# RWails/shadow

Hardware: AMD Instinct MI355X
Metric: SSSP source-paths/sec + attached-pair matrix build time; % HBM peak, 1/2/4/8 GPU (higher is better)
Workload: dtype f64

## Files before the change

### include/shadowtopo.h

```cpp
#ifndef SHADOWTOPO_H
#define SHADOWTOPO_H

#include <stddef.h>
#include <stdint.h>

#ifdef __cplusplus
extern "C" {
#endif

typedef struct shadowtopo_engine shadowtopo_engine;

#define SHADOWTOPO_OK 0
#define SHADOWTOPO_EINVAL (-1)
#define SHADOWTOPO_ENOMEM (-2)
#define SHADOWTOPO_EDEVICE (-3)
#define SHADOWTOPO_ESTATE (-4)
#define SHADOWTOPO_EINTERNAL (-5)

#define SHADOWTOPO_F_DIRECTED 0x1u
#define SHADOWTOPO_F_COMPLETE 0x2u
#define SHADOWTOPO_F_PREFER_DIRECT 0x4u
#define SHADOWTOPO_F_SELF_DIJKSTRA_LOOP 0x8u
#define SHADOWTOPO_F_AUTO_COMPLETE 0x10u
#define SHADOWTOPO_F_FORCE_DENSE 0x20u
#define SHADOWTOPO_F_FORCE_CSR 0x40u

#define SHADOWTOPO_MEM_HOST 0
#define SHADOWTOPO_MEM_DEVICE 1
#define SHADOWTOPO_MEM_HOST_LR 2

#define SHADOWTOPO_KIND_NONE 0
#define SHADOWTOPO_KIND_DIRECT 1
#define SHADOWTOPO_KIND_SELF 2
#define SHADOWTOPO_KIND_DIJKSTRA 3

#define SHADOWTOPO_OPT_BATCHES_IN_FLIGHT 1
#define SHADOWTOPO_OPT_TIMING 2
#define SHADOWTOPO_OPT_MAX_ROUNDS 3
#define SHADOWTOPO_OPT_FORCE_REPLAY 4
#define SHADOWTOPO_OPT_PROFILE 5
#define SHADOWTOPO_OPT_DENSE_VARIANT 6
#define SHADOWTOPO_DENSE_F32 0
#define SHADOWTOPO_DENSE_F64 1
#define SHADOWTOPO_OPT_DELTA_PERMILLE 7
#define SHADOWTOPO_OPT_CSR_VARIANT 8
#define SHADOWTOPO_OPT_DENSE_BATCHES_PER_WAVE 9
#define SHADOWTOPO_OPT_SOURCE_ORDER 10
#define SHADOWTOPO_OPT_DENSE_SEED 11
#define SHADOWTOPO_OPT_DENSE_PRUNE 12

#define SHADOWTOPO_OPT_WORKLIST 14
#define SHADOWTOPO_OPT_GRID_X 15
#define SHADOWTOPO_OPT_PRUNE_PENDANT 16
#define SHADOWTOPO_OPT_DEVICE_ROUNDS 17
#define SHADOWTOPO_OPT_DELTA_LIVE 19
#define SHADOWTOPO_OPT_DENSE_W16 20
#define SHADOWTOPO_OPT_SWEEP_PARTS 22
#define SHADOWTOPO_OPT_CHAIN_PARTS 23
#define SHADOWTOPO_OPT_DENSE_SPEC 21
#define SHADOWTOPO_OPT_HEAVY_FIRST 27
#define SHADOWTOPO_OPT_WALK_TPW 28
#define SHADOWTOPO_OPT_CSR_LEAN 30
#define SHADOWTOPO_OPT_CSR_INCREMENTAL 31
#define SHADOWTOPO_OPT_SPEC_COMPOSE 33
#define SHADOWTOPO_OPT_SPIN_US 35
#define SHADOWTOPO_OPT_HOST_GROUPS 36
#define SHADOWTOPO_OPT_SWEEP_STATS 37
#define SHADOWTOPO_OPT_SWEEP_WINDOWS 38
#define SHADOWTOPO_OPT_SWEEP_GLDS 39
#define SHADOWTOPO_OPT_SWEEP_REFILTER 40
#define SHADOWTOPO_OPT_SWEEP_WAVES 41
#define SHADOWTOPO_OPT_SEED_SKIP 42
#define SHADOWTOPO_OPT_DELTA_W16 43
#define SHADOWTOPO_OPT_PART0_PERMILLE 29
#define SHADOWTOPO_OPT_TEST_UNCONVERGED 24
#define SHADOWTOPO_OPT_TEST_SCRAMBLE_TREE 25
#define SHADOWTOPO_OPT_TEST_POOL_ENOMEM 26
#define SHADOWTOPO_OPT_HBM_SHARE 13

#define SHADOWTOPO_CSR_FULL 1
#define SHADOWTOPO_CSR_PUSH 2

typedef struct shadowtopo_stats {
    int64_t n_vertices;
    int64_t n_edges;
    int64_t n_arcs;
    int64_t n_attached;
    int64_t sources;
    int64_t batches;
    int64_t rounds;
    int64_t relax_launches;
    int64_t replayed_sources;
    int64_t tainted_pairs;
    double relax_ms;
    double compose_ms;
    double replay_ms;
    double wall_ms;
    int32_t device;
    int32_t multigraph;
    int32_t dense;
    int32_t reserved;
    int64_t visits;
    int64_t changes;
    int64_t full_sweeps;
    int64_t delta_sweeps;
    double full_ms;
    double delta_ms;
    int64_t full_batches;
    int64_t full_changes;
    int64_t relax_batches;
    int64_t wl_launches;
    double wl_ms;
    int64_t sparse_deltas;
    double self_ms;
    int64_t self_paths;
    int64_t pruned_deltas;
    int64_t pruned_vertices;
    int64_t pool_allocs;
    double pool_alloc_ms;
    double create_validate_ms;
    double create_upload_ms;
    double create_build_ms;
    double order_ms;
    double create_alloc_ms;
// ... 76 lines not shown
```

### shadow_amd/csrc/engine.hip

```cpp
#include <hip/hip_runtime.h>
#include <sys/mman.h>

#include <algorithm>
#include <atomic>
#include <chrono>
#include <cmath>
#include <cstdarg>
#include <cstdint>
#include <cstdlib>
#include <cstdio>
#include <cstring>
#include <functional>
#include <limits>
#include <mutex>
#include <string>
#include <thread>
#include <type_traits>
#include <vector>

#include "graph_build.h"
#include "shadowtopo.h"

namespace {

// ... 1499 lines not shown
                    int nr = 0;
#pragma unroll
                    for (int x = 0; x < XR; ++x) {
                        rp[x] = u0;
                        if (hrows) {
                            rp[x] = u0 + __builtin_ctzll(hrows);
                            hrows &= hrows - 1;
                            nr = x + 1;
                        }
                        ur[x] = PR ? perm[rp[x]] : rp[x];
                    }
                    double d64[XR], ws[XR][TDT];
#pragma unroll
                    for (int x = 0; x < XR; ++x) {
                        d64[x] = (lpass >> (rp[x] - u0)) & 1ull ? Dl[(size_t)ur[x] * KL] : dinf();
#pragma unroll
                        for (int t = 0; t < TDT; ++t) ws[x][t] = W[(size_t)rp[x] * Vp + v0 + t];
                    }
#pragma unroll
                    for (int x = 0; x < XR; ++x) {
                        if (x >= nr) break;
                        const int32_t u = ur[x];
                        const bool own = (u == sv[k]);
#pragma unroll
                        for (int t = 0; t < TDT; ++t) {
                            const double c = d64[x] + ws[x][t];
                            if (__ballot((c <= bc[k][t]) & !own)) {
                                if (!own) lex_update(c, d64[x], u, bc[k][t], bdu[k][t], bu[k][t], tie[k], 1u << t);
                            }
                        }
                    }
                }
            }
        }
    }
    if (v0 < V) {
#pragma unroll
        for (int k = 0; k < TB; ++k)
            if (live[k])
            {
                SeedRows sr;
                if (PR && WIp && sv[k] >= 0) {
                    sr.WIp = WIp;
                    sr.WRp = WRp;
                    sr.srow = (size_t)ipos[sv[k]] * Vp;
                    sr.rs = vfac[sv[k]];
                }
                dense_epilogue<TDT>(B[k], lane, sv[k], v0, V, bc[k], bdu[k], bu[k], tie[k], WI, Vp, in_r, parity,
                                    cnt, b0 + k, vid, sr,
                                    mdc_out ? mdc_out + ((size_t)(b0 + k) * (Vp / KL) + v0 / KL) * KL : nullptr,
                                    seeded != 0);
            }
    }
}

constexpr int HEAVY_MAX = 2048;
struct HeavyArgs {
    const uint32_t* w[4];
    int32_t* o[4];
    int32_t slots[4];
};
__global__ __launch_bounds__(1024) void k_heavy_order(HeavyArgs ha) {
    __shared__ unsigned long long key[HEAVY_MAX];
    const int x = blockIdx.x, part = blockIdx.y;
    const int32_t S = ha.slots[part];
    if (S <= 0) return;
    const uint32_t* w = ha.w[part];
    int32_t* ord = ha.o[part];
    int n2 = 1;
    while (n2 < S) n2 <<= 1;
    for (int j = threadIdx.x; j < n2; j += blockDim.x)
        key[j] = j < S ? ((unsigned long long)w[8 * j + x] << 32) | (uint32_t)(0xffffffffu - (uint32_t)j) : 0ull;
    __syncthreads();
    for (int k = 2; k <= n2; k <<= 1)
        for (int jj = k >> 1; jj > 0; jj >>= 1) {
            for (int i = threadIdx.x; i < n2; i += blockDim.x) {
                const int l = i ^ jj;
                if (l > i) {
                    const unsigned long long a = key[i], b = key[l];
                    const bool desc = (i & k) == 0;
                    if (desc ? a < b : a > b) {
                        key[i] = b;
                        key[l] = a;
                    }
                }
            }
            __syncthreads();
        }
    for (int r = threadIdx.x; r < S; r += blockDim.x) {
        const int32_t j = (int32_t)(0xffffffffu - (uint32_t)key[r]);
        ord[8 * r + x] = 8 * j + x;
    }
}

template <typename T>
__global__ __launch_bounds__(256) void k_permute_w(const T* __restrict__ W, const int32_t* __restrict__ perm,
                                                   int32_t Vp, T* __restrict__ Wp) {
    const size_t i = blockIdx.x;
    const __attribute__((address_space(1))) T* src = (const __attribute__((address_space(1))) T*)W + (size_t)perm[i] * Vp;
    for (int32_t j = threadIdx.x; j < Vp; j += 256) Wp[i * Vp + j] = src[perm[j]];
}

__global__ __launch_bounds__(256) void k_w16(const float* __restrict__ W32p, uint16_t* __restrict__ W16p, size_t n) {
    for (size_t i = (size_t)blockIdx.x * blockDim.x + threadIdx.x; i < n; i += (size_t)gridDim.x * blockDim.x) {
        const float f = W32p[i];
        uint16_t hb;
// ... 1430 lines not shown
    void* stage = nullptr;
    size_t stage_bytes = 0;
    hipStream_t copy_stream = nullptr;
    hipEvent_t ev_comp[2] = {nullptr, nullptr}, ev_copy[2] = {nullptr, nullptr};
    ReplayDev rp{};
    bool rp_ready = false;
    std::vector<void*> rp_allocs;
    int32_t opt_nb = 0;
    int32_t opt_timing = 0;
    int64_t opt_max_rounds = 0;
    int32_t opt_force_replay = 0;
    int32_t opt_profile = 0;
    int32_t opt_dense_variant = 0;
    int32_t opt_dense_tb = 1;
    int32_t opt_delta_permille = 125;
    int32_t opt_hbm_share = 1000;
    bool floor_ok = false;
    bool floor_checked = false;
    size_t pool_bytes = 0;
    int32_t opt_worklist = 1;
    int32_t opt_csr_variant = SHADOWTOPO_CSR_FULL;
    int32_t trace_rounds = 0;
    int32_t opt_delta_live = 2;
    int32_t opt_delta_live_div = 64;
    int32_t opt_delta_colbound = 2;
    int32_t opt_sweep_spiral = 1;
    int32_t opt_sweep_win1 = 8;
    int32_t opt_sweep_split = 1;
    int32_t opt_sweep_parts = 2;
    hipStream_t aux_stream[3] = {nullptr, nullptr, nullptr};
    hipEvent_t ev_h0 = nullptr, ev_hp[3] = {nullptr, nullptr, nullptr};
    hipEvent_t ev_sw[4] = {nullptr, nullptr, nullptr, nullptr};
    int32_t opt_chain_parts = 1;
    int32_t opt_fuse_mindc = 1;
    int32_t opt_part0_permille = 562;
    int32_t opt_host_split = 4;
    int64_t opt_grid_x = (int64_t)1 << 23;
    int32_t* d_live = nullptr;
    int32_t* d_nlive = nullptr;
    unsigned long long* d_prof = nullptr;
    unsigned long long* prof_buf = nullptr;
    hipEvent_t ev0 = nullptr, ev1 = nullptr, evm = nullptr, evm2 = nullptr;
    hipEvent_t ev_spin = nullptr;
    std::vector<hipEvent_t> ev_dev;
    std::vector<hipEvent_t> ev_spec;
    void* d_pk_scratch = nullptr;
    size_t pk_scratch_n = 0;
    int32_t* h_cnt_spec = nullptr;
    int32_t opt_dense_spec = 2;
    int32_t opt_sweep_glds = 0;
    int32_t opt_sweep_stats = 0;
    unsigned long long* d_sweep_hits = nullptr;
    int32_t opt_sweep_waves = 4;
    int32_t opt_sweep_refilter = 0;
    int32_t opt_seed_skip = 1;
    int32_t opt_delta_w16 = 1;
    float* d_thrio = nullptr;
    size_t thrio_n = 0;
    int32_t opt_heavy_first = 1;
    int32_t opt_csr_lean = 2;
    bool lean_next = false;
    ViewBufs vb;
    size_t view_cap_a = 0;
    int32_t opt_host_groups = 0;
    int32_t opt_spin_us = 20000;
    int32_t opt_spec_compose = 1;
    unsigned long long* h_masks = nullptr;
    size_t h_masks_n = 0;
    int32_t opt_csr_incremental = 32;
    int32_t opt_walk_tpw = 1;
    uint32_t* d_bweight[4] = {nullptr, nullptr, nullptr, nullptr};
    int32_t* d_border[4][2] = {};
    size_t heavy_cap[4] = {0, 0, 0, 0};
    int64_t heavy_key[4] = {-1, -1, -1, -1};
    int64_t heavy_next[4] = {-1, -1, -1, -1};
    int heavy_buf = 0;
    int32_t opt_test_unconverged = 0;
    int32_t opt_test_scramble = 0;
    int32_t opt_test_pool_enomem = 0;
    bool unconverged = false;
    shadowtopo_stats st{};
};

namespace {

int dev_alloc(std::vector<void*>& owner, void** p, size_t bytes) {
    if (bytes == 0) bytes = 8;
    hipError_t e = hipMalloc(p, bytes);
    if (e != hipSuccess) return fail(SHADOWTOPO_ENOMEM, "hipMalloc(%zu): %s", bytes, hipGetErrorString(e));
    owner.push_back(*p);
    return SHADOWTOPO_OK;
}

template <typename T>
int upload(shadowtopo_engine* eng, const std::vector<T>& h, const T** out) {
    void* p = nullptr;
    int rc = dev_alloc(eng->graph_allocs, &p, h.size() * sizeof(T));
    if (rc) return rc;
    if (!h.empty()) HIP_TRY(hipMemcpy(p, h.data(), h.size() * sizeof(T), hipMemcpyHostToDevice));
    *out = static_cast<const T*>(p);
    return SHADOWTOPO_OK;
}

float f32_round_down(double x) {
    float f = (float)x;
    if ((double)f > x) f = std::nextafter(f, -std::numeric_limits<float>::infinity());
// ... 214 lines not shown
                           float* mdc_out, int32_t seeded) {
    constexpr int TDT = FTDT, XR = 2;
    const int32_t ntb = (eng->V + 4 * TDT - 1) / (4 * TDT);
    const int32_t ngroups = (nbg + TB - 1) / TB;
    const int64_t nblocks = 8 * (((int64_t)ngroups * ntb + 7) / 8);
    const size_t nchunks = (size_t)((eng->V + SRS - 1) / SRS);
    const size_t need = (size_t)ngroups * (size_t)(eng->Vp / TDT) * TB * nchunks;
    if (eng->hitlog_n < need) {
        if (eng->d_hitlog) (void)hipFree(eng->d_hitlog);
        eng->d_hitlog = nullptr;
        eng->hitlog_n = 0;
        hipError_t e = hipMalloc((void**)&eng->d_hitlog, need * sizeof(uint32_t));
        if (e != hipSuccess) return e;
        eng->hitlog_n = need;
    }
    if (eng->vperm_ready && eng->opt_dense_prune) {
        const size_t mneed = (size_t)eng->nb_cap * nchunks * KL;
        if (eng->minD_n < mneed) {
            if (eng->d_minD) (void)hipFree(eng->d_minD);
            eng->d_minD = nullptr;
            eng->minD_n = 0;
            hipError_t e = hipMalloc((void**)&eng->d_minD, mneed * sizeof(float));
            if (e != hipSuccess) return e;
            eng->minD_n = mneed;
        }
        hipLaunchKernelGGL(k_min_d32, dim3((uint32_t)((nchunks + 3) / 4), nbg), dim3(256), 0, s, eng->pools,
                           eng->d_perm, (int32_t)nchunks, eng->d_minD);
        if (TB <= 2 && eng->opt_sweep_split) {
            if (eng->opt_dense_w16) {
                hipError_t e = ensure_w16p(eng, s);
                if (e != hipSuccess) return e;
            }
            bool w16 = false;
            if constexpr (TB == 1 && TDT == 8) {
                w16 = eng->opt_dense_w16 != 0;
                if (w16)
                    hipLaunchKernelGGL((k_relax_dense_f<TDT, XR, TB, true, 1, 4, true>), dim3((uint32_t)nblocks), dim3(256),
                                       0, s, (const float*)eng->d_W16p, eng->d_Wp, eng->d_WI, eng->Vp, eng->g.in_r,
                                       eng->pools, eng->V, nbg, ntb, par, thresh, cnt_prev, cnt_cur, eng->d_prof,
                                       eng->d_hitlog, eng->d_perm, eng->d_minW, eng->d_minD, eng->d_pos, eng->d_WIp,
                                       eng->d_WRp, eng->g.vfac, eng->opt_sweep_spiral, eng->opt_sweep_win1, nullptr);
            }
            if constexpr (TB == 1) {
                const int32_t parts = sweep_parts(eng, nbg);
                if (!w16 && parts >= 2 && !eng->d_prof) {
                    hipError_t e = hipSuccess;
                    if (!eng->ev_h0) e = hipEventCreateWithFlags(&eng->ev_h0, hipEventDisableTiming);
                    for (int k = 0; k < parts - 1 && e == hipSuccess; ++k) {
                        if (!eng->aux_stream[k]) e = hipStreamCreateWithFlags(&eng->aux_stream[k], hipStreamNonBlocking);
                        if (e == hipSuccess && !eng->ev_hp[k]) e = hipEventCreateWithFlags(&eng->ev_hp[k], hipEventDisableTiming);
                    }
                    if (e == hipSuccess && mdc_out)
                        e = hipMemsetD32Async((hipDeviceptr_t)mdc_out, 0x7fc00000, (size_t)nbg * (eng->Vp / KL) * KL, s);
                    if (e == hipSuccess) e = hipEventRecord(eng->ev_h0, s);
                    for (int k = 0; k < parts - 1 && e == hipSuccess; ++k) e = hipStreamWaitEvent(eng->aux_stream[k], eng->ev_h0, 0);
                    if (e != hipSuccess) return e;
                    if (eng->opt_sweep_stats && !eng->d_sweep_hits &&
                        (e = hipMalloc((void**)&eng->d_sweep_hits, 2 * sizeof(unsigned long long))) != hipSuccess)
                        return e;
                    if (eng->opt_sweep_stats && (e = hipMemsetAsync(eng->d_sweep_hits, 0, 2 * sizeof(unsigned long long), s)) != hipSuccess)
                        return e;
                    if (eng->opt_sweep_refilter) {
                        const size_t need_t = (size_t)nbg * eng->Vp * KL;
                        if (eng->thrio_n < need_t) {
                            if (eng->d_thrio) (void)hipFree(eng->d_thrio);
                            eng->d_thrio = nullptr;
                            eng->thrio_n = 0;
                            if ((e = hipMalloc((void**)&eng->d_thrio, need_t * sizeof(float))) != hipSuccess) return e;
                            eng->thrio_n = need_t;
                        }
                    }
                    const int cur = eng->heavy_buf;
                    HeavyArgs ha{};
                    bool sort_any = false;
                    auto part = [&](hipStream_t st, int32_t b0, int32_t n, int k) {
                        const Pools P = pools_from(eng->pools, b0);
                        uint32_t* hl = eng->d_hitlog + (size_t)b0 * (size_t)(eng->Vp / TDT) * nchunks;
                        const float* mD = eng->d_minD + (size_t)b0 * nchunks * KL;
                        const int64_t nbl = 8 * (((int64_t)n * ntb + 7) / 8);
                        const bool w8 = eng->opt_sweep_waves == 8;
                        const int32_t ntb1 = w8 ? (eng->V + 8 * TDT - 1) / (8 * TDT) : ntb;
                        const int64_t nbl1 = 8 * (((int64_t)n * ntb1 + 7) / 8);
                        const int64_t key = ((int64_t)b0 << 42) | ((int64_t)n << 21) | ((int64_t)w8 << 20) | ntb1;
                        bool heavy = eng->opt_heavy_first && k < 4 && nbl1 / 8 <= HEAVY_MAX;
                        if (heavy && eng->heavy_cap[k] < (size_t)nbl1) {
                            for (void* q : {(void*)eng->d_bweight[k], (void*)eng->d_border[k][0], (void*)eng->d_border[k][1]})
                                if (q) (void)hipFree(q);
                            eng->d_bweight[k] = nullptr;
                            eng->d_border[k][0] = eng->d_border[k][1] = nullptr;
                            eng->heavy_cap[k] = 0;
                            eng->heavy_key[k] = -1;
                            if (hipMalloc((void**)&eng->d_bweight[k], sizeof(uint32_t) * nbl1) != hipSuccess ||
                                hipMalloc((void**)&eng->d_border[k][0], sizeof(int32_t) * nbl1) != hipSuccess ||
                                hipMalloc((void**)&eng->d_border[k][1], sizeof(int32_t) * nbl1) != hipSuccess ||
                                hipMemsetAsync(eng->d_bweight[k], 0, sizeof(uint32_t) * nbl1, st) != hipSuccess) {
                                (void)hipGetLastError();
                                heavy = false;
                            } else {
                                eng->heavy_cap[k] = (size_t)nbl1;
                            }
                        }
                        const int32_t* ord = heavy && eng->heavy_key[k] == key ? eng->d_border[k][cur] : nullptr;
                        float* tio = eng->opt_sweep_refilter ? eng->d_thrio + (size_t)b0 * eng->Vp * KL : nullptr;
                        if (w8 && eng->opt_sweep_glds)
                            hipLaunchKernelGGL((k_relax_dense_f<TDT, XR, 1, true, 1, 8, false, true>), dim3((uint32_t)nbl1),
                                               dim3(512), 0, st, eng->d_W32p, eng->d_Wp, eng->d_WI, eng->Vp, eng->g.in_r,
                                               P, eng->V, n, ntb1, par, thresh, cnt_prev + b0, cnt_cur + b0, nullptr, hl,
                                               eng->d_perm, eng->d_minW, mD, eng->d_pos, eng->d_WIp, eng->d_WRp,
                                               eng->g.vfac, eng->opt_sweep_spiral, eng->opt_sweep_win1, nullptr, ord,
                                               heavy ? eng->d_bweight[k] : nullptr, tio);
                        else if (w8)
                            hipLaunchKernelGGL((k_relax_dense_f<TDT, XR, 1, true, 1, 8, false, false>), dim3((uint32_t)nbl1),
                                               dim3(512), 0, st, eng->d_W32p, eng->d_Wp, eng->d_WI, eng->Vp, eng->g.in_r,
                                               P, eng->V, n, ntb1, par, thresh, cnt_prev + b0, cnt_cur + b0, nullptr, hl,
                                               eng->d_perm, eng->d_minW, mD, eng->d_pos, eng->d_WIp, eng->d_WRp,
                                               eng->g.vfac, eng->opt_sweep_spiral, eng->opt_sweep_win1, nullptr, ord,
                                               heavy ? eng->d_bweight[k] : nullptr, tio);
                        else if (eng->opt_sweep_glds)
                            hipLaunchKernelGGL((k_relax_dense_f<TDT, XR, 1, true, 1, 4, false, true>), dim3((uint32_t)nbl),
                                               dim3(256), 0, st, eng->d_W32p, eng->d_Wp, eng->d_WI, eng->Vp, eng->g.in_r,
                                               P, eng->V, n, ntb, par, thresh, cnt_prev + b0, cnt_cur + b0, nullptr, hl,
                                               eng->d_perm, eng->d_minW, mD, eng->d_pos, eng->d_WIp, eng->d_WRp,
                                               eng->g.vfac, eng->opt_sweep_spiral, eng->opt_sweep_win1, nullptr, ord,
                                               heavy ? eng->d_bweight[k] : nullptr, tio);
                        else
                        hipLaunchKernelGGL((k_relax_dense_f<TDT, XR, 1, true, 1>), dim3((uint32_t)nbl), dim3(256), 0, st,
                                           eng->d_W32p, eng->d_Wp, eng->d_WI, eng->Vp, eng->g.in_r, P, eng->V, n, ntb,
                                           par, thresh, cnt_prev + b0, cnt_cur + b0, nullptr, hl, eng->d_perm,
                                           eng->d_minW, mD, eng->d_pos, eng->d_WIp, eng->d_WRp, eng->g.vfac,
                                           eng->opt_sweep_spiral, eng->opt_sweep_win1, nullptr, ord,
                                           heavy ? eng->d_bweight[k] : nullptr, tio);
                        if (heavy) {
                            ha.w[k] = eng->d_bweight[k];
                            ha.o[k] = eng->d_border[k][cur ^ 1];
                            ha.slots[k] = (int32_t)(nbl1 / 8);
                            eng->heavy_next[k] = key;
                            sort_any = true;
                        } else {
                            eng->heavy_next[k] = -1;
                        }
                        hipLaunchKernelGGL((k_relax_dense_f<TDT, XR, 1, true, 2>), dim3((uint32_t)nbl), dim3(256), 0, st,
                                           eng->d_W32p, eng->d_Wp, eng->d_WI, eng->Vp, eng->g.in_r, P, eng->V, n, ntb,
                                           par, thresh, cnt_prev + b0, cnt_cur + b0,
                                           eng->opt_sweep_stats ? eng->d_sweep_hits : nullptr, hl, eng->d_perm,
                                           eng->d_minW, mD, eng->d_pos, eng->d_WIp, eng->d_WRp, eng->g.vfac,
                                           eng->opt_sweep_spiral, eng->opt_sweep_win1,
                                           mdc_out ? mdc_out + (size_t)b0 * (eng->Vp / KL) * KL : nullptr, nullptr,
                                           nullptr, tio, seeded);
                        if (tail && e == hipSuccess) e = (*tail)(st, b0, n, k);
                    };
                    auto bound = [&](int k) {
                        if (parts == 2 && k == 1 && eng->opt_part0_permille > 0)
                            return std::max<int32_t>(1, std::min<int32_t>(nbg - 1, (int32_t)(((int64_t)nbg * eng->opt_part0_permille + 500) / 1000)));
                        return (int32_t)((int64_t)nbg * k / parts);
                    };
                    for (int k = 0; k < parts; ++k) {
                        const int32_t b0 = bound(k), b1 = bound(k + 1);
                        part(k == 0 ? s : eng->aux_stream[k - 1], b0, b1 - b0, k);
                    }
                    if (sort_any && e == hipSuccess) {
                        hipLaunchKernelGGL(k_heavy_order, dim3(8, (uint32_t)std::min(parts, 4)), dim3(1024), 0, s, ha);
                        for (int k = 0; k < 4; ++k) eng->heavy_key[k] = k < parts ? eng->heavy_next[k] : -1;
                        eng->heavy_buf = cur ^ 1;
                    }
                    for (int k = 0; k < parts - 1 && e == hipSuccess; ++k) {
                        e = hipEventRecord(eng->ev_hp[k], eng->aux_stream[k]);
                        if (e == hipSuccess) e = hipStreamWaitEvent(s, eng->ev_hp[k], 0);
                    }
                    if (e != hipSuccess) return e;
                    if (eng->opt_sweep_stats && sort_any) {
                        if ((e = hipStreamSynchronize(s)) != hipSuccess) return e;
                        for (int k = 0; k < parts && k < 4; ++k) {
                            if (!ha.w[k]) continue;
                            std::vector<uint32_t> wk((size_t)ha.slots[k] * 8);
                            if ((e = hipMemcpy(wk.data(), ha.w[k], wk.size() * sizeof(uint32_t), hipMemcpyDeviceToHost)) != hipSuccess)
                                return e;
                            for (uint32_t x : wk) eng->st.sweep_chunks += x;
                            const int32_t ntbs = eng->opt_sweep_waves == 8 ? (eng->V + 8 * TDT - 1) / (8 * TDT) : ntb;
                            eng->st.sweep_chunk_slots += (int64_t)(bound(k + 1) - bound(k)) * ntbs * (int64_t)nchunks;
                        }
                        unsigned long long hits = 0;
                        if ((e = hipMemcpy(&hits, eng->d_sweep_hits, sizeof hits, hipMemcpyDeviceToHost)) != hipSuccess) return e;
                        eng->st.sweep_hit_rows += (int64_t)hits;
                    }
                    return hipGetLastError();
                }
            }
            if (!w16)
            hipLaunchKernelGGL((k_relax_dense_f<TDT, XR, TB, true, 1>), dim3((uint32_t)nblocks), dim3(256), 0, s,
                               eng->d_W32p, eng->d_Wp, eng->d_WI, eng->Vp, eng->g.in_r, eng->pools, eng->V, nbg, ntb,
                               par, thresh, cnt_prev, cnt_cur, eng->d_prof, eng->d_hitlog, eng->d_perm, eng->d_minW,
                               eng->d_minD, eng->d_pos, eng->d_WIp, eng->d_WRp, eng->g.vfac, eng->opt_sweep_spiral,
                               eng->opt_sweep_win1, nullptr);
            const int64_t nblocks1 = 8 * (((int64_t)nbg * ntb + 7) / 8);
            hipLaunchKernelGGL((k_relax_dense_f<TDT, XR, 1, true, 2>), dim3((uint32_t)nblocks1), dim3(256), 0, s,
                               eng->d_W32p, eng->d_Wp, eng->d_WI, eng->Vp, eng->g.in_r, eng->pools, eng->V, nbg, ntb,
                               par, thresh, cnt_prev, cnt_cur, eng->d_prof, eng->d_hitlog, eng->d_perm, eng->d_minW,
                               eng->d_minD, eng->d_pos, eng->d_WIp, eng->d_WRp, eng->g.vfac, eng->opt_sweep_spiral,
                               eng->opt_sweep_win1, nullptr, nullptr, nullptr, nullptr, seeded);
            return hipGetLastError();
        }
        hipLaunchKernelGGL((k_relax_dense_f<TDT, XR, TB, true>), dim3((uint32_t)nblocks), dim3(256), 0, s,
                           eng->d_W32p, eng->d_Wp, eng->d_WI, eng->Vp, eng->g.in_r, eng->pools, eng->V, nbg, ntb, par,
                           thresh, cnt_prev, cnt_cur, eng->d_prof, eng->d_hitlog, eng->d_perm, eng->d_minW,
                           eng->d_minD, eng->d_pos, eng->d_WIp, eng->d_WRp, eng->g.vfac, eng->opt_sweep_spiral,
                               eng->opt_sweep_win1, nullptr);
        return hipGetLastError();
    }
    hipLaunchKernelGGL((k_relax_dense_f<TDT, XR, TB, false>), dim3((uint32_t)nblocks), dim3(256), 0, s, eng->d_W32,
                       eng->d_W, eng->d_WI, eng->Vp, eng->g.in_r, eng->pools, eng->V, nbg, ntb, par, thresh, cnt_prev,
                       cnt_cur, eng->d_prof, eng->d_hitlog, nullptr, nullptr, nullptr, nullptr, nullptr, nullptr, nullptr, 0, 0, nullptr);
    return hipGetLastError();
}

hipError_t launch_dense_f(shadowtopo_engine* eng, int32_t nbg, int32_t par, int32_t thresh,
                          const int32_t* cnt_prev, int32_t* cnt_cur, hipStream_t s, const PartTail* tail = nullptr,
                          float* mdc_out = nullptr, bool seeded = false) {
    const int32_t sd = seeded && eng->opt_seed_skip;
    switch (eng->opt_dense_tb) {
        case 1: return launch_dense_ft<1>(eng, nbg, par, thresh, cnt_prev, cnt_cur, s, tail, mdc_out, sd);
        case 4: return launch_dense_ft<4>(eng, nbg, par, thresh, cnt_prev, cnt_cur, s, tail, mdc_out, sd);
        default: return launch_dense_ft<2>(eng, nbg, par, thresh, cnt_prev, cnt_cur, s, tail, mdc_out, sd);
    }
}

bool delta_is_sparse(const shadowtopo_engine* eng, int32_t nbg, int32_t thresh) {
    if (eng->opt_delta_live != 2) return eng->opt_delta_live == 1;
    int64_t dch = 0, dpairs = 0;
    for (int32_t b = 0; b < nbg; ++b)
        if (eng->h_cnt[b] > 0 && eng->h_cnt[b] <= thresh) {
            dch += eng->h_cnt[b];
// ... 2047 lines not shown
        case SHADOWTOPO_OPT_SWEEP_PARTS:
            if (value < 1 || value > 4) return fail(SHADOWTOPO_EINVAL, "sweep parts must be 1 .. 4");
            eng->opt_sweep_parts = (int32_t)value;
            return SHADOWTOPO_OK;
        case SHADOWTOPO_OPT_DENSE_SPEC:
            if (value < 0 || value > SPEC_MAX) return fail(SHADOWTOPO_EINVAL, "dense spec rounds must be in [0, 4]");
            eng->opt_dense_spec = (int32_t)value;
            return SHADOWTOPO_OK;
        case SHADOWTOPO_OPT_DELTA_LIVE:
            if (value < 0 || value > 2) return fail(SHADOWTOPO_EINVAL, "delta live must be 0, 1 or 2");
            eng->opt_delta_live = (int32_t)value;
            return SHADOWTOPO_OK;
        case SHADOWTOPO_OPT_WORKLIST:
            if (value < 0 || value > 2) return fail(SHADOWTOPO_EINVAL, "worklist must be 0, 1 or 2");
            eng->opt_worklist = (int32_t)value;
            return SHADOWTOPO_OK;
        case SHADOWTOPO_OPT_HBM_SHARE:
            if (value < 1 || value > 1000) return fail(SHADOWTOPO_EINVAL, "HBM share must be in [1, 1000] per mille");
            eng->opt_hbm_share = (int32_t)value;
            return SHADOWTOPO_OK;
        case SHADOWTOPO_OPT_CSR_LEAN:
            if (value < 0 || value > 2) return fail(SHADOWTOPO_EINVAL, "CSR lean must be 0, 1 or 2");
            eng->opt_csr_lean = (int32_t)value;
            return SHADOWTOPO_OK;
        case SHADOWTOPO_OPT_HOST_GROUPS:
            if (value < 0 || value > 1024) return fail(SHADOWTOPO_EINVAL, "host groups must be in [0, 1024]");
            eng->opt_host_groups = (int32_t)value;
            return SHADOWTOPO_OK;
        case SHADOWTOPO_OPT_SWEEP_WINDOWS:
            if (value < 0 || (value & 0xff) >= 64 || ((value >> 8) & 0xff) >= 64 || value >= (1 << 16))
                return fail(SHADOWTOPO_EINVAL, "sweep windows: bits 0-7 and 8-15 must each be in [0, 63]");
            eng->opt_sweep_win1 = (int32_t)value;
            return SHADOWTOPO_OK;
        case SHADOWTOPO_OPT_SWEEP_GLDS:
            if (value != 0 && value != 1) return fail(SHADOWTOPO_EINVAL, "sweep glds must be 0 or 1");
            eng->opt_sweep_glds = (int32_t)value;
            return SHADOWTOPO_OK;
        case SHADOWTOPO_OPT_SWEEP_WAVES:
            if (value != 4 && value != 8) return fail(SHADOWTOPO_EINVAL, "sweep waves must be 4 or 8");
            eng->opt_sweep_waves = (int32_t)value;
            return SHADOWTOPO_OK;
        case SHADOWTOPO_OPT_DELTA_W16:
            if (value != 0 && value != 1) return fail(SHADOWTOPO_EINVAL, "delta w16 must be 0 or 1");
            eng->opt_delta_w16 = (int32_t)value;
            return SHADOWTOPO_OK;
        case SHADOWTOPO_OPT_SEED_SKIP:
            if (value != 0 && value != 1) return fail(SHADOWTOPO_EINVAL, "seed skip must be 0 or 1");
            eng->opt_seed_skip = (int32_t)value;
            return SHADOWTOPO_OK;
        case SHADOWTOPO_OPT_SWEEP_REFILTER:
            if (value != 0 && value != 1) return fail(SHADOWTOPO_EINVAL, "sweep refilter must be 0 or 1");
            eng->opt_sweep_refilter = (int32_t)value;
            return SHADOWTOPO_OK;
        case SHADOWTOPO_OPT_SWEEP_STATS:
            eng->opt_sweep_stats = value ? 1 : 0;
            return SHADOWTOPO_OK;
        case SHADOWTOPO_OPT_SPIN_US:
            if (value < 0 || value > 10000000) return fail(SHADOWTOPO_EINVAL, "spin must be in [0, 1e7] us");
            eng->opt_spin_us = (int32_t)value;
            return SHADOWTOPO_OK;
        case SHADOWTOPO_OPT_SPEC_COMPOSE:
            if (value != 0 && value != 1) return fail(SHADOWTOPO_EINVAL, "speculative compose must be 0 or 1");
            eng->opt_spec_compose = (int32_t)value;
            return SHADOWTOPO_OK;
        case SHADOWTOPO_OPT_CSR_INCREMENTAL:
            if (value < 0 || value > (1 << 20)) return fail(SHADOWTOPO_EINVAL, "CSR incremental must be in [0, 2^20]");
            eng->opt_csr_incremental = (int32_t)value;
            return SHADOWTOPO_OK;
        case SHADOWTOPO_OPT_PART0_PERMILLE:
            if (value < 1 || value > 999) return fail(SHADOWTOPO_EINVAL, "part 0 share must be in [1, 999] per mille");
            eng->opt_part0_permille = (int32_t)value;
            return SHADOWTOPO_OK;
        case SHADOWTOPO_OPT_WALK_TPW:
            if (value < 1 || value > 4) return fail(SHADOWTOPO_EINVAL, "walk shape must be 1 .. 4");
            eng->opt_walk_tpw = (int32_t)value;
            return SHADOWTOPO_OK;
        case SHADOWTOPO_OPT_HEAVY_FIRST:
            if (value != 0 && value != 1) return fail(SHADOWTOPO_EINVAL, "heavy first must be 0 or 1");
            eng->opt_heavy_first = (int32_t)value;
            return SHADOWTOPO_OK;
        case SHADOWTOPO_OPT_TEST_UNCONVERGED:
            eng->opt_test_unconverged = value ? 1 : 0;
            return SHADOWTOPO_OK;
        case SHADOWTOPO_OPT_TEST_POOL_ENOMEM:
            eng->opt_test_pool_enomem = value ? 1 : 0;
            return SHADOWTOPO_OK;
        case SHADOWTOPO_OPT_TEST_SCRAMBLE_TREE:
            if (value < 0 || value > 2) return fail(SHADOWTOPO_EINVAL, "scramble mode must be 0, 1 or 2");
            eng->opt_test_scramble = (int32_t)value;
            return SHADOWTOPO_OK;
        case SHADOWTOPO_OPT_DELTA_PERMILLE:
            if (value < 0 || value > 1000) return fail(SHADOWTOPO_EINVAL, "delta per mille must be in [0, 1000]");
            eng->opt_delta_permille = (int32_t)value;
            return SHADOWTOPO_OK;
        default:
            return fail(SHADOWTOPO_EINVAL, "unknown option %d", key);
    }
}

int shadowtopo_compute_rows(shadowtopo_engine* eng, int32_t row_begin, int32_t row_end, double* lat, double* rel,
                            uint32_t* hops, uint8_t* kind, int32_t mem, void* stream) {
    if (!eng) return fail(SHADOWTOPO_EINVAL, "NULL engine");
    if (!eng->d_attached) return fail(SHADOWTOPO_ESTATE, "shadowtopo_set_attached not called");
    if (row_begin < 0 || row_end > eng->A || row_begin > row_end) return fail(SHADOWTOPO_EINVAL, "bad row range");
    if (row_begin == row_end) return SHADOWTOPO_OK;
    if (mem != SHADOWTOPO_MEM_HOST && mem != SHADOWTOPO_MEM_DEVICE && mem != SHADOWTOPO_MEM_HOST_LR)
// ... 478 lines not shown
```

### shadow_amd/engine.py

```python
from __future__ import annotations

import ctypes
import os

import numpy as np

HERE = os.path.dirname(os.path.abspath(__file__))
LIB_PATH = os.environ.get("SHADOWTOPO_EXP_LIB") or os.path.join(HERE, "_build", "libshadowtopo_hip.so")

F_DIRECTED = 0x1
F_COMPLETE = 0x2
F_PREFER_DIRECT = 0x4
F_SELF_DIJKSTRA_LOOP = 0x8
F_AUTO_COMPLETE = 0x10
F_FORCE_DENSE = 0x20
F_FORCE_CSR = 0x40

MEM_HOST = 0
MEM_DEVICE = 1
MEM_HOST_LR = 2

KIND_NONE, KIND_DIRECT, KIND_SELF, KIND_DIJKSTRA = 0, 1, 2, 3

OPT_BATCHES_IN_FLIGHT = 1
OPT_TIMING = 2
OPT_MAX_ROUNDS = 3
OPT_FORCE_REPLAY = 4
OPT_PROFILE = 5
OPT_DENSE_VARIANT = 6
DENSE_F32 = 0
DENSE_F64 = 1
OPT_DELTA_PERMILLE = 7
OPT_CSR_VARIANT = 8
OPT_DENSE_BATCHES_PER_WAVE = 9
OPT_SOURCE_ORDER = 10
OPT_DENSE_SEED = 11
OPT_DENSE_PRUNE = 12
OPT_HBM_SHARE = 13
OPT_WORKLIST = 14
OPT_GRID_X = 15
OPT_PRUNE_PENDANT = 16
OPT_DEVICE_ROUNDS = 17
OPT_DENSE_W16 = 20
OPT_CHAIN_PARTS = 23
OPT_SWEEP_PARTS = 22
OPT_DENSE_SPEC = 21
OPT_DELTA_LIVE = 19
OPT_WALK_TPW = 28
OPT_CSR_LEAN = 30
OPT_CSR_INCREMENTAL = 31
OPT_SPEC_COMPOSE = 33
OPT_SPIN_US = 35
OPT_HOST_GROUPS = 36
OPT_SWEEP_WINDOWS = 38
OPT_SWEEP_GLDS = 39
OPT_SWEEP_REFILTER = 40
OPT_SWEEP_WAVES = 41
OPT_DELTA_W16 = 43
OPT_SEED_SKIP = 42
OPT_SWEEP_STATS = 37
OPT_PART0_PERMILLE = 29
OPT_HEAVY_FIRST = 27
OPT_TEST_UNCONVERGED = 24
OPT_TEST_SCRAMBLE_TREE = 25
OPT_TEST_POOL_ENOMEM = 26
CSR_FULL = 1
CSR_PUSH = 2

ENGINE_SYMBOLS = (
    "shadowtopo_device_count", "shadowtopo_prepare", "shadowtopo_last_error", "shadowtopo_create", "shadowtopo_destroy",
    "shadowtopo_set_attached", "shadowtopo_set_option", "shadowtopo_compute_rows", "shadowtopo_sssp",
    "shadowtopo_get_stats", "shadowtopo_reset_stats", "shadowtopo_is_complete", "shadowtopo_get_eid",
    "shadowtopo_host_alloc", "shadowtopo_host_free", "shadowtopo_self_rule_paths",
    "shadowtopo_packed_capacity", "shadowtopo_pack_rows", "shadowtopo_unpack_rows",
    "shadowtopo_hops_narrow", "shadowtopo_hops_widen",
)


class ShadowTopoError(RuntimeError):
    pass


class Stats(ctypes.Structure):
    _fields_ = [
        ("n_vertices", ctypes.c_int64), ("n_edges", ctypes.c_int64), ("n_arcs", ctypes.c_int64),
        ("n_attached", ctypes.c_int64), ("sources", ctypes.c_int64), ("batches", ctypes.c_int64),
        ("rounds", ctypes.c_int64), ("relax_launches", ctypes.c_int64), ("replayed_sources", ctypes.c_int64),
        ("tainted_pairs", ctypes.c_int64), ("relax_ms", ctypes.c_double), ("compose_ms", ctypes.c_double),
        ("replay_ms", ctypes.c_double), ("wall_ms", ctypes.c_double), ("device", ctypes.c_int32),
        ("multigraph", ctypes.c_int32), ("dense", ctypes.c_int32), ("reserved", ctypes.c_int32),
        ("visits", ctypes.c_int64), ("changes", ctypes.c_int64),
        ("full_sweeps", ctypes.c_int64), ("delta_sweeps", ctypes.c_int64),
        ("full_ms", ctypes.c_double), ("delta_ms", ctypes.c_double),
        ("full_batches", ctypes.c_int64), ("full_changes", ctypes.c_int64), ("relax_batches", ctypes.c_int64),
        ("wl_launches", ctypes.c_int64), ("wl_ms", ctypes.c_double), ("sparse_deltas", ctypes.c_int64),
        ("self_ms", ctypes.c_double), ("self_paths", ctypes.c_int64), ("pruned_deltas", ctypes.c_int64),
        ("pruned_vertices", ctypes.c_int64), ("pool_allocs", ctypes.c_int64), ("pool_alloc_ms", ctypes.c_double),
        ("create_validate_ms", ctypes.c_double), ("create_upload_ms", ctypes.c_double),
        ("create_build_ms", ctypes.c_double), ("order_ms", ctypes.c_double),
        ("create_alloc_ms", ctypes.c_double), ("groups", ctypes.c_int64),
        ("prepare_ms", ctypes.c_double), ("create_prepare_wait_ms", ctypes.c_double),
        ("group_batches", ctypes.c_int64), ("host_syncs", ctypes.c_int64),
        ("push_ms", ctypes.c_double), ("pred_ms", ctypes.c_double), ("fold_ms", ctypes.c_double),
        ("push_rounds", ctypes.c_int64), ("fold_rounds", ctypes.c_int64),
        ("packed_pairs", ctypes.c_int64), ("packed_explicit", ctypes.c_int64),
        ("compose_kernel_ms", ctypes.c_double), ("walk_targets", ctypes.c_int64),
        ("attach_prep_ms", ctypes.c_double), ("lean_groups", ctypes.c_int64),
        ("spec_composes", ctypes.c_int64), ("spec_composes_lost", ctypes.c_int64),
        ("sweep_chunks", ctypes.c_int64), ("sweep_chunk_slots", ctypes.c_int64), ("sweep_hit_rows", ctypes.c_int64),
# ... 247 lines not shown
```

Baseline: 333,300.

## Add destination-lane dense sweep kernel mapping lanes to destinations by default

Adds a new dense sweep kernel in which each wave lane owns a destination vertex and loops over a few sources, instead of lanes over sources. Blocks cover 32 sources by 64 destinations, with W and D chunks double-buffered in LDS and chunk-level pruning done through ballots. The aim is to skip more chunk work by changing the shape of the live region and to raise reuse of W rows per wave. It is enabled by default through a new option; the hit log now has to be zeroed before each sweep, and the new kernel uses different threshold, register and LDS behaviour.

After: 372,600, median of 6. +11.8%, better.

```diff
diff --git a/_exp/sweep_lane_shape_sim.py b/_exp/sweep_lane_shape_sim.py
--- /dev/null
+++ b/_exp/sweep_lane_shape_sim.py
@@ -0,0 +1,113 @@
+import sys
+
+import numpy as np
+
+sys.path.insert(0, ".")
+from shadow_amd import synth
+
+V = int(sys.argv[1]) if len(sys.argv) > 1 else 10_000
+A = V // 10
+SRS, KL = 32, 64
+nb = (A + KL - 1) // KL
+BATCHES = [int(x) for x in sys.argv[2].split(",")] if len(sys.argv) > 2 else sorted({0, nb // 2, nb - 2 if nb > 2 else nb - 1})
+
+
+def hilbert(x, y, n=1 << 12):
+    x = (x * (n - 1)).astype(np.int64)
+    y = (y * (n - 1)).astype(np.int64)
+    dd = np.zeros_like(x)
+    s = n >> 1
+    while s > 0:
+        rx = ((x & s) > 0).astype(np.int64)
+        ry = ((y & s) > 0).astype(np.int64)
+        dd += s * s * ((3 * rx) ^ ry)
+        m = ry == 0
+        f = m & (rx == 1)
+        x = np.where(f, n - 1 - x, x)
+        y = np.where(f, n - 1 - y, y)
+        x2 = np.where(m, y, x)
+        y = np.where(m, x, y)
+        x = x2
+        s >>= 1
+    return dd
+
+
+g = synth.geometric_complete_ish(V=V, A=A)
+pts = np.random.default_rng(1).random((V, 2))
+perm = np.argsort(hilbert(pts[:, 0], pts[:, 1]), kind="stable")
+pos = np.empty(V, np.int64)
+pos[perm] = np.arange(V)
+W = np.full((V, V), np.inf, np.float32)
+src, dst = pos[np.asarray(g.src)], pos[np.asarray(g.dst)]
+lat = np.asarray(g.latency, np.float32)
+keep = src != dst
+W[src[keep], dst[keep]] = lat[keep]
+if not g.directed:
+    W = np.minimum(W, W.T)
+att = np.sort(pos[np.asarray(g.attached)])
+nchunks = (V + SRS - 1) // SRS
+Vc = nchunks * SRS
+Vt = (V + KL - 1) // KL * KL
+Wr = np.full((Vc, V), np.inf, np.float32)
+Wr[:V] = W
+minW = Wr.reshape(nchunks, SRS, V).min(1)
+del Wr
+
+
+def min_plus(D):
+    out = D.copy()
+    tmp = np.empty((1024, V), np.float32)
+    for s in range(D.shape[0]):
+        for u0 in range(0, V, 1024):
+            n = min(1024, V - u0)
+            np.add(W[u0:u0 + n], D[s, u0:u0 + n, None], out=tmp[:n])
+            np.minimum(out[s], tmp[:n].min(0), out=out[s])
+    return out
+
+
+SHAPES = [("wave 64 x 8, block 64 x 32 (source lanes)", 64, 8, 64, 32),
+          ("wave 8 x 64, block 32 x 64 (destination lanes)", 8, 64, 32, 64),
+          ("wave 16 x 32", 16, 32, None, None),
+          ("wave 32 x 16", 32, 16, None, None),
+          ("single pairs (floor of any box bound)", 1, 1, None, None)]
+acc = {name: [0, 0, 0, 0] for name, *_ in SHAPES}
+for b in BATCHES:
+    S = att[b * KL:(b + 1) * KL]
+    ns = len(S)
+    D0 = np.full((KL, V), np.inf, np.float32)
+    D0[:ns] = W[S]
+    thr = D0.copy()
+    thr[np.arange(ns), S] = 0.0
+    thr = min_plus(min_plus(thr))
+    thr[np.arange(ns), S] = -np.inf
+    thr[ns:] = -np.inf
+    D0r = np.full((KL, Vc), np.inf, np.float32)
+    D0r[:, :V] = D0
+    minD = D0r.reshape(KL, nchunks, SRS).min(2)
+    thr_p = np.full((KL, Vt), -np.inf, np.float32)
+    thr_p[:, :V] = thr * np.float32(1 + 1e-6)
+    minW_p = np.full((nchunks, Vt), np.inf, np.float32)
+    minW_p[:, :V] = minW
+    live = np.empty((nchunks, KL, Vt), bool)
+    for c in range(nchunks):
+        live[c] = minD[:, c, None] + minW_p[c][None, :] <= thr_p
+    ntiles = {gt: (V + gt - 1) // gt for gt in (1, 8, 16, 32, 64)}
+    for name, gs, gt, bs, bt in SHAPES:
+        w = live.reshape(nchunks, KL // gs, gs, Vt // gt, gt).any(axis=(2, 4))[:, :, :ntiles[gt]]
+        acc[name][0] += int(w.sum())
+        acc[name][1] += w.size
+        if bs:
+            bl = live.reshape(nchunks, KL // bs, bs, Vt // bt, bt).any(axis=(2, 4))[:, :, :ntiles[bt]]
+            acc[name][2] += int(bl.sum())
+            acc[name][3] += bl.size
+    print(f"batch {b}: {ns} sources done", file=sys.stderr, flush=True)
+
+print(f"C2 generator, V = {V}, A = {A}, batches {BATCHES} of {nb}, every tile, {nchunks} chunks of {SRS} rows")
+print(f"{'shape (sources x destinations)':50s} {'live (wave, chunk)':>19s} {'live (block, chunk)':>20s} {'waves per staged chunk':>23s}")
+for name, *_ in SHAPES:
+    lw, sw, lb, sb = acc[name]
+    fw = lw / sw
+    if sb:
+        print(f"{name:50s} {fw:19.3f} {lb / sb:20.3f} {fw / (lb / sb):23.2f}")
+    else:
+        print(f"{name:50s} {fw:19.3f}")
diff --git a/include/shadowtopo.h b/include/shadowtopo.h
--- a/include/shadowtopo.h
+++ b/include/shadowtopo.h
@@ -70,6 +70,7 @@
 #define SHADOWTOPO_OPT_SWEEP_GLDS 39
 #define SHADOWTOPO_OPT_SWEEP_REFILTER 40
 #define SHADOWTOPO_OPT_SWEEP_WAVES 41
+#define SHADOWTOPO_OPT_SWEEP_LANES 44
 #define SHADOWTOPO_OPT_SEED_SKIP 42
 #define SHADOWTOPO_OPT_DELTA_W16 43
 #define SHADOWTOPO_OPT_PART0_PERMILLE 29
diff --git a/shadow_amd/csrc/engine.hip b/shadow_amd/csrc/engine.hip
--- a/shadow_amd/csrc/engine.hip
+++ b/shadow_amd/csrc/engine.hip
@@ -1575,6 +1575,252 @@
                                     seeded != 0);
             }
     }
+}
+
+__global__ __launch_bounds__(256) __attribute__((amdgpu_waves_per_eu(6))) void k_sweep_dest_lanes(
+    const float* __restrict__ W32p, const double* __restrict__ Wp, int32_t Vp, Pools pools, int32_t V, int32_t nb,
+    int32_t ntl, int32_t thresh, const int32_t* __restrict__ cnt_prev, uint32_t* __restrict__ hitlog,
+    const int32_t* __restrict__ perm, const float* __restrict__ minW, const float* __restrict__ minD,
+    const int32_t* __restrict__ ipos, int32_t spiral, int32_t win1, const int32_t* __restrict__ border,
+    uint32_t* __restrict__ bweight) {
+    constexpr int NT = 256, SO = 8;
+    constexpr int BS = 32, BD = 64;
+    struct SweepLds {
+        float d[2][SRS * BS];
+        float w[2][SRS * BD];
+        unsigned long long win[2];
+    };
+    __shared__ __attribute__((aligned(16))) SweepLds slds;
+    auto& sD = slds.d;
+    auto& sW = slds.w;
+    auto& sWin = slds.win;
+    const int64_t Lb = border ? (int64_t)border[blockIdx.x] : (int64_t)blockIdx.x;
+    int32_t b, it;
+    if (!xcd_tile(Lb, nb, 2 * ntl, b, it)) return;
+    const int32_t h = it & 1, t0 = (it >> 1) * BD;
+    if (!(cnt_prev[b] > thresh) || t0 >= V) {
+        if (bweight && threadIdx.x == 0) bweight[Lb] = 0u;
+        return;
+    }
+    const int32_t wave = __builtin_amdgcn_readfirstlane(threadIdx.x >> 6);
+    const int lane = threadIdx.x & 63;
+    const int32_t s0 = BS * h + SO * wave;
+    const int32_t p = t0 + lane;
+    const BatchDev B = batch_view(pools, b);
+    float thr[SO];
+    {
+        const int32_t v = perm[p];
+        double cd[SO];
+#pragma unroll
+        for (int j = 0; j < SO; ++j) cd[j] = B.D[(size_t)v * KL + s0 + j];
+#pragma unroll
+        for (int j = 0; j < SO; ++j) {
+            const int32_t sj = B.srcv[s0 + j];
+            const double ws = (sj >= 0 && sj != v) ? Wp[(size_t)ipos[sj >= 0 ? sj : 0] * Vp + p] : dinf();
+            const double bc = ws < dinf() ? 0.0 + ws : dmax();
+            thr[j] = sj >= 0 && p < V ? f32_thr(cd[j] < bc ? cd[j] : bc) : __int_as_float(0x7fc00000);
+        }
+    }
+    const int32_t nrows = (V + SRS - 1) / SRS * SRS;
+    const int32_t nchunks = nrows / SRS;
+    typedef float f4 __attribute__((ext_vector_type(4)));
+    typedef __attribute__((address_space(1))) const f4 gf4;
+    constexpr int WQ = BD / 4;
+    constexpr int DQ4 = BS / 4;
+    constexpr int WQT = SRS * WQ / NT;
+    static_assert(SRS * DQ4 == NT && WQT * NT == SRS * WQ, "one D32 piece and whole W32p pieces per thread");
+    f4 pd, pw[WQT];
+    float mdn[SO], mdc[SO], mwn, mwc;
+    const gfloat* mDb = (const gfloat*)minD + (size_t)b * nchunks * KL + s0;
+    const gfloat* mWl = (const gfloat*)minW + p;
+    const int32_t c0 = (int32_t)((int64_t)t0 / SRS % nchunks);
+    const int32_t sL = c0, sR = nchunks - 1 - c0, sM = sL < sR ? sL : sR;
+    auto chunk_of = [&](int32_t j) {
+        if (!spiral) return (c0 + j) % nchunks;
+        if (j <= 2 * sM) return j == 0 ? c0 : ((j & 1) ? c0 + (j + 1) / 2 : c0 - j / 2);
+        return sR > sL ? c0 + j - sM : c0 - (j - sM);
+    };
+    auto perm_of = [&](int32_t j) { return perm[chunk_of(j) * SRS + (int)threadIdx.x / DQ4]; };
+    auto fetch = [&](int32_t j, int32_t prow) {
+        const int32_t c = chunk_of(j);
+        const int32_t u0 = c * SRS;
+        pd = *(gf4*)(B.D32 + (size_t)prow * KL + BS * h + ((int)threadIdx.x % DQ4) * 4);
+#pragma unroll
+        for (int j2 = 0; j2 < SO; ++j2) mdn[j2] = mDb[(size_t)c * KL + j2];
+        mwn = mWl[(size_t)c * Vp];
+#pragma unroll
+        for (int i = 0; i < WQT; ++i) {
+            const int e = threadIdx.x + i * NT;
+            pw[i] = *(gf4*)((const gfloat*)W32p + (size_t)(u0 + e / WQ) * Vp + t0 + (e % WQ) * 4);
+        }
+    };
+    auto stash = [&](int buf) {
+        *(f4*)&sD[buf][threadIdx.x * 4] = pd;
+#pragma unroll
+        for (int i = 0; i < WQT; ++i) *(f4*)&sW[buf][(threadIdx.x + i * NT) * 4] = pw[i];
+    };
+    auto advance = [&]() {
+#pragma unroll
+        for (int j = 0; j < SO; ++j) mdc[j] = mdn[j];
+        mwc = mwn;
+    };
+    if (threadIdx.x == 0) sWin[0] = sWin[1] = 0ull;
+    __syncthreads();
+    int32_t cur_win = -1;
+    unsigned long long cur_live = 0ull;
+    const int32_t w1 = (win1 & 0xff) < 64 ? (win1 & 0xff) : 0;
+    const int32_t wf = ((win1 >> 8) & 0xff) > 0 && ((win1 >> 8) & 0xff) < 64 ? (win1 >> 8) & 0xff : 64;
+    auto win_of = [&](int32_t j) {
+        if (j == 0) return 0;
+        if (w1) return j <= w1 ? 1 : 2 + (j - 1 - w1) / wf;
+        return 1 + (j - 1) / wf;
+    };
+    auto win_base = [&](int32_t wi) {
+        if (wi == 0) return 0;
+        if (w1) return wi == 1 ? 1 : 1 + w1 + (wi - 2) * wf;
+        return 1 + (wi - 1) * wf;
+    };
+    auto win_size = [&](int32_t wi) { return wi == 0 ? 1 : (w1 && wi == 1 ? w1 : wf); };
+    constexpr int WG = 4;
+    auto eval_window = [&](int32_t wi) -> unsigned long long {
+        const int32_t base = win_base(wi);
+        const int32_t nw = nchunks - base < win_size(wi) ? nchunks - base : win_size(wi);
+        unsigned long long wm = 0ull;
+        const int32_t cl = chunk_of(base + (lane < nw ? lane : 0));
+        for (int32_t j0 = 0; j0 < nw; j0 += WG) {
+            float md[WG][SO], mw[WG];
+#pragma unroll
+            for (int jj = 0; jj < WG; ++jj) {
+                const int32_t c = __builtin_amdgcn_readlane(cl, j0 + jj < nw ? j0 + jj : 0);
+#pragma unroll
+                for (int j = 0; j < SO; ++j) md[jj][j] = mDb[(size_t)c * KL + j];
+                mw[jj] = mWl[(size_t)c * Vp];
+            }
+#pragma unroll
+            for (int jj = 0; jj < WG; ++jj) {
+                float tm = thr[0] - md[jj][0];
+#pragma unroll
+                for (int j = 1; j < SO; ++j) tm = fmaxf(tm, thr[j] - md[jj][j]);
+                if (__ballot(mw[jj] <= tm) && j0 + jj < nw) wm |= 1ull << (j0 + jj);
+            }
+        }
+        if (threadIdx.x == 0) sWin[(wi + 1) & 1] = 0ull;
+        if (lane == 0 && wm) atomicOr(&sWin[wi & 1], wm);
+        __syncthreads();
+        return ((unsigned long long)(uint32_t)__builtin_amdgcn_readfirstlane((int)(uint32_t)(sWin[wi & 1] >> 32)) << 32) |
+               (uint32_t)__builtin_amdgcn_readfirstlane((int)(uint32_t)sWin[wi & 1]);
+    };
+    auto next_live = [&](int32_t from) -> int32_t {
+        while (from < nchunks) {
+            const int32_t wi = win_of(from);
+            if (wi != cur_win) {
+                cur_win = wi;
+                cur_live = eval_window(wi);
+            }
+            const unsigned long long m = cur_live & (~0ull << (from - win_base(wi)));
+            if (m) return win_base(wi) + __builtin_ctzll(m);
+            from = win_base(wi + 1);
+        }
+        return -1;
+    };
+    uint32_t* hl = hitlog + ((size_t)b * (size_t)(Vp / 8) + (size_t)(p / 8)) * nchunks;
+    int32_t prow_n = 0;
+    uint32_t nvis = 0;
+    int32_t itc = next_live(0);
+    if (itc >= 0) {
+        prow_n = perm_of(itc);
+        fetch(itc, prow_n);
+        stash(0);
+        advance();
+    }
+    int32_t itn = itc >= 0 ? next_live(itc + 1) : -1;
+    if (itn >= 0) prow_n = perm_of(itn);
+    __syncthreads();
+    int bufc = 0;
+    while (itc >= 0) {
+        const int32_t c = chunk_of(itc);
+        const int cur = bufc;
+        const bool more = itn >= 0;
+        if (more) fetch(itn, prow_n);
+        const int32_t itn2 = more ? next_live(itn + 1) : -1;
+        if (itn2 >= 0) prow_n = perm_of(itn2);
+        bool run;
+        {
+            float tm = thr[0] - mdc[0];
+#pragma unroll
+            for (int j = 1; j < SO; ++j) tm = fmaxf(tm, thr[j] - mdc[j]);
+            run = __ballot(mwc <= tm) != 0;
+        }
+        uint32_t hits = 0;
+        typedef __attribute__((address_space(3))) const f4 lf4;
+        typedef __attribute__((address_space(3))) const float lf1;
+        uint32_t wbase = (uint32_t)(uintptr_t)(lf1*)&sW[cur][lane];
+        uint32_t dbase = (uint32_t)(uintptr_t)(lf4*)&sD[cur][SO * wave];
+        asm volatile("" : "+v"(wbase), "+v"(dbase));
+        float wn;
+        f4 dn[SO / 4];
+        auto lds_row = [&](int r) {
+            wn = *(lf1*)(uintptr_t)(wbase + (uint32_t)(r * BD) * 4u);
+#pragma unroll
+            for (int j = 0; j < SO / 4; ++j) dn[j] = *(lf4*)(uintptr_t)(dbase + (uint32_t)(r * BS + 4 * j) * 4u);
+        };
+        if (run) lds_row(0);
+#pragma unroll 8
+        for (int r = 0; r < (run ? SRS : 0); ++r) {
+            const float w = wn;
+            f4 d4[SO / 4];
+#pragma unroll
+            for (int j = 0; j < SO / 4; ++j) d4[j] = dn[j];
+            if (r + 1 < SRS) lds_row(r + 1);
+            typedef float f2 __attribute__((ext_vector_type(2)));
+            float x[SO];
+#pragma unroll
+            for (int j = 0; j < SO / 4; ++j) {
+                const f2 a = f2{thr[4 * j], thr[4 * j + 1]} - f2{d4[j].x, d4[j].y};
+                const f2 e = f2{thr[4 * j + 2], thr[4 * j + 3]} - f2{d4[j].z, d4[j].w};
+                x[4 * j] = a.x;
+                x[4 * j + 1] = a.y;
+                x[4 * j + 2] = e.x;
+                x[4 * j + 3] = e.y;
+            }
+            float g = fmaxf(fmaxf(x[0], x[1]), x[2]);
+#pragma unroll
+            for (int t = 3; t + 1 < SO; t += 2) g = fmaxf(fmaxf(g, x[t]), x[t + 1]);
+            g = fmaxf(g, x[SO - 1]);
+            const bool pass = w <= g;
+            if (__ballot(pass)) {
+                hits |= pass ? 1u << r : 0u;
+#pragma unroll
+                for (int j = 0; j < SO / 4; ++j) {
+                    const float dj[4] = {d4[j].x, d4[j].y, d4[j].z, d4[j].w};
+#pragma unroll
+                    for (int i = 0; i < 4; ++i) {
+                        const float c32 = dj[i] + w;
+                        const float nbd = __int_as_float(__float_as_int(c32) + 9);
+                        float& th = thr[4 * j + i];
+                        th = ((c32 < __int_as_float(0x7f800000)) & (nbd < th)) ? nbd : th;
+                    }
+                }
+            }
+        }
+        if (__ballot(hits != 0u)) {
+            uint32_t h8 = hits;
+            h8 |= (uint32_t)__shfl_xor((int)h8, 1);
+            h8 |= (uint32_t)__shfl_xor((int)h8, 2);
+            h8 |= (uint32_t)__shfl_xor((int)h8, 4);
+            if ((lane & 7) == 0 && h8) atomicOr(hl + c, h8);
+        }
+        if (more) {
+            stash(cur ^ 1);
+            advance();
+        }
+        __syncthreads();
+        bufc ^= 1;
+        itc = itn;
+        itn = itn2;
+        ++nvis;
+    }
+    if (bweight && threadIdx.x == 0) bweight[Lb] = nvis;
 }
 
 constexpr int HEAVY_MAX = 2048;
@@ -3111,6 +3357,7 @@
     int32_t opt_sweep_stats = 0;
     unsigned long long* d_sweep_hits = nullptr;
     int32_t opt_sweep_waves = 4;
+    int32_t opt_sweep_lanes = 1;
     int32_t opt_sweep_refilter = 0;
     int32_t opt_seed_skip = 1;
     int32_t opt_delta_w16 = 1;
@@ -3431,14 +3678,17 @@
                     }
                     if (e == hipSuccess && mdc_out)
                         e = hipMemsetD32Async((hipDeviceptr_t)mdc_out, 0x7fc00000, (size_t)nbg * (eng->Vp / KL) * KL, s);
+                    if (e == hipSuccess && eng->opt_sweep_stats && !eng->d_sweep_hits)
+                        e = hipMalloc((void**)&eng->d_sweep_hits, 2 * sizeof(unsigned long long));
+                    if (e == hipSuccess && eng->opt_sweep_stats)
+                        e = hipMemsetAsync(eng->d_sweep_hits, 0, 2 * sizeof(unsigned long long), s);
+                    const bool dest_lanes = eng->opt_sweep_lanes && eng->opt_sweep_waves != 8 && !eng->opt_sweep_glds &&
+                                            !eng->opt_sweep_refilter;
+                    if (e == hipSuccess && dest_lanes)
+                        e = hipMemsetAsync(eng->d_hitlog, 0, (size_t)nbg * (size_t)(eng->Vp / TDT) * nchunks * sizeof(uint32_t), s);
                     if (e == hipSuccess) e = hipEventRecord(eng->ev_h0, s);
                     for (int k = 0; k < parts - 1 && e == hipSuccess; ++k) e = hipStreamWaitEvent(eng->aux_stream[k], eng->ev_h0, 0);
                     if (e != hipSuccess) return e;
-                    if (eng->opt_sweep_stats && !eng->d_sweep_hits &&
-                        (e = hipMalloc((void**)&eng->d_sweep_hits, 2 * sizeof(unsigned long long))) != hipSuccess)
-                        return e;
-                    if (eng->opt_sweep_stats && (e = hipMemsetAsync(eng->d_sweep_hits, 0, 2 * sizeof(unsigned long long), s)) != hipSuccess)
-                        return e;
                     if (eng->opt_sweep_refilter) {
                         const size_t need_t = (size_t)nbg * eng->Vp * KL;
                         if (eng->thrio_n < need_t) {
@@ -3450,6 +3700,7 @@
                         }
                     }
                     const int cur = eng->heavy_buf;
+                    const int32_t ntl = (eng->V + KL - 1) / KL;
                     HeavyArgs ha{};
                     bool sort_any = false;
                     auto part = [&](hipStream_t st, int32_t b0, int32_t n, int k) {
@@ -3458,9 +3709,11 @@
                         const float* mD = eng->d_minD + (size_t)b0 * nchunks * KL;
                         const int64_t nbl = 8 * (((int64_t)n * ntb + 7) / 8);
                         const bool w8 = eng->opt_sweep_waves == 8;
-                        const int32_t ntb1 = w8 ? (eng->V + 8 * TDT - 1) / (8 * TDT) : ntb;
+                        const bool dl = dest_lanes;
+                        const int32_t ntb1 = dl ? 2 * ntl : w8 ? (eng->V + 8 * TDT - 1) / (8 * TDT) : ntb;
                         const int64_t nbl1 = 8 * (((int64_t)n * ntb1 + 7) / 8);
-                        const int64_t key = ((int64_t)b0 << 42) | ((int64_t)n << 21) | ((int64_t)w8 << 20) | ntb1;
+                        const int64_t key = ((int64_t)b0 << 42) | ((int64_t)n << 21) | ((int64_t)w8 << 20) |
+                                            ((int64_t)dl << 19) | ntb1;
                         bool heavy = eng->opt_heavy_first && k < 4 && nbl1 / 8 <= HEAVY_MAX;
                         if (heavy && eng->heavy_cap[k] < (size_t)nbl1) {
                             for (void* q : {(void*)eng->d_bweight[k], (void*)eng->d_border[k][0], (void*)eng->d_border[k][1]})
@@ -3481,7 +3734,12 @@
                         }
                         const int32_t* ord = heavy && eng->heavy_key[k] == key ? eng->d_border[k][cur] : nullptr;
                         float* tio = eng->opt_sweep_refilter ? eng->d_thrio + (size_t)b0 * eng->Vp * KL : nullptr;
-                        if (w8 && eng->opt_sweep_glds)
+                        if (dl)
+                            hipLaunchKernelGGL(k_sweep_dest_lanes, dim3((uint32_t)nbl1), dim3(256), 0, st, eng->d_W32p,
+                                               eng->d_Wp, eng->Vp, P, eng->V, n, ntl, thresh, cnt_prev + b0, hl,
+                                               eng->d_perm, eng->d_minW, mD, eng->d_pos, eng->opt_sweep_spiral,
+                                               eng->opt_sweep_win1, ord, heavy ? eng->d_bweight[k] : nullptr);
+                        else if (w8 && eng->opt_sweep_glds)
                             hipLaunchKernelGGL((k_relax_dense_f<TDT, XR, 1, true, 1, 8, false, true>), dim3((uint32_t)nbl1),
                                                dim3(512), 0, st, eng->d_W32p, eng->d_Wp, eng->d_WI, eng->Vp, eng->g.in_r,
                                                P, eng->V, n, ntb1, par, thresh, cnt_prev + b0, cnt_cur + b0, nullptr, hl,
@@ -3547,15 +3805,15 @@
                         if (e == hipSuccess) e = hipStreamWaitEvent(s, eng->ev_hp[k], 0);
                     }
                     if (e != hipSuccess) return e;
-                    if (eng->opt_sweep_stats && sort_any) {
+                    if (eng->opt_sweep_stats) {
                         if ((e = hipStreamSynchronize(s)) != hipSuccess) return e;
-                        for (int k = 0; k < parts && k < 4; ++k) {
+                        for (int k = 0; k < parts && k < 4 && sort_any; ++k) {
                             if (!ha.w[k]) continue;
                             std::vector<uint32_t> wk((size_t)ha.slots[k] * 8);
                             if ((e = hipMemcpy(wk.data(), ha.w[k], wk.size() * sizeof(uint32_t), hipMemcpyDeviceToHost)) != hipSuccess)
                                 return e;
                             for (uint32_t x : wk) eng->st.sweep_chunks += x;
-                            const int32_t ntbs = eng->opt_sweep_waves == 8 ? (eng->V + 8 * TDT - 1) / (8 * TDT) : ntb;
+                            const int32_t ntbs = dest_lanes ? 2 * ntl : eng->opt_sweep_waves == 8 ? (eng->V + 8 * TDT - 1) / (8 * TDT) : ntb;
                             eng->st.sweep_chunk_slots += (int64_t)(bound(k + 1) - bound(k)) * ntbs * (int64_t)nchunks;
                         }
                         unsigned long long hits = 0;
@@ -5709,6 +5967,10 @@
             if (value != 0 && value != 1) return fail(SHADOWTOPO_EINVAL, "sweep refilter must be 0 or 1");
             eng->opt_sweep_refilter = (int32_t)value;
             return SHADOWTOPO_OK;
+        case SHADOWTOPO_OPT_SWEEP_LANES:
+            if (value != 0 && value != 1) return fail(SHADOWTOPO_EINVAL, "sweep lanes must be 0 or 1");
+            eng->opt_sweep_lanes = (int32_t)value;
+            return SHADOWTOPO_OK;
         case SHADOWTOPO_OPT_SWEEP_STATS:
             eng->opt_sweep_stats = value ? 1 : 0;
             return SHADOWTOPO_OK;
diff --git a/shadow_amd/engine.py b/shadow_amd/engine.py
--- a/shadow_amd/engine.py
+++ b/shadow_amd/engine.py
@@ -55,6 +55,7 @@
 OPT_SWEEP_WINDOWS = 38
 OPT_SWEEP_GLDS = 39
 OPT_SWEEP_REFILTER = 40
+OPT_SWEEP_LANES = 44
 OPT_SWEEP_WAVES = 41
 OPT_DELTA_W16 = 43
 OPT_SEED_SKIP = 42
```
